# 23skdu/longbow

Hardware: AMD Instinct MI355X
Metric: k-NN queries/sec (batch=1024, k=100), 1Mx768 f32 (higher is better)
Workload: dtype f32

## Files before the change

### longbow_amd/build.py

```python
import os
import subprocess
import sys
from concurrent.futures import ThreadPoolExecutor

HERE = os.path.dirname(os.path.abspath(__file__))
CSRC = os.path.join(HERE, "csrc")
OUT = os.path.join(HERE, "liblongbow_gpu.so")
OUT_DIAG = os.path.join(HERE, "liblongbow_gpu_diag.so")
SOURCES = ["index.hip", "index_search.hip", "simd_api.hip", "pq.hip", "comm.hip", "flight.hip", "kernels_gemm.hip", "kernels_gemm_narrow.hip", "kernels_gemm_tall2.hip", "kernels_gemm_tall16.hip", "kernels_scan.hip", "kernels_select.hip", "kernels_finish.hip",
           "kernels_pq.hip", "kernels_pq2.hip", "kernels_filter.hip", "kernels_i8.hip"]
HEADERS = ["lb_device.h", "lb_exact.h", "lb_admit.h", "lb_host.h", "lb_index.h", "lb_combine.h", "lb_select.h", os.path.join("..", "..", "include", "longbow_gpu.h")]
HIPCC = os.environ.get("HIPCC", "/opt/rocm/bin/hipcc")
FLAGS = ["--offload-arch=gfx950", "-O3", "-std=c++17", "-fPIC", "-Wall", "-Wno-unused-function"]


def _stale(target, deps):
    if not os.path.exists(target):
        return True
    t = os.path.getmtime(target)
    return any(os.path.getmtime(d) > t for d in deps)


def build(force=False, verbose=False, diag=False):
    srcs = [s for s in SOURCES if os.path.exists(os.path.join(CSRC, s))]
    hdrs = [os.path.join(CSRC, h) for h in HEADERS]
    objs = []
    jobs = []
    out = OUT_DIAG if diag else OUT
    for s in srcs:
        src = os.path.join(CSRC, s)
        obj = os.path.join(CSRC, s.replace(".hip", ".diag.o" if diag else ".o"))
        objs.append(obj)
        if force or _stale(obj, [src] + hdrs):
            jobs.append([HIPCC] + FLAGS + (["-DLB_DIAG"] if diag else []) + ["-c", src, "-o", obj])

    def run(cmd):
        if verbose:
            print(" ".join(cmd), flush=True)
        r = subprocess.run(cmd, capture_output=True, text=True)
        if r.returncode != 0:
            raise RuntimeError("hipcc failed:\n" + " ".join(cmd) + "\n" + r.stdout + r.stderr)
        return r

    with ThreadPoolExecutor(max_workers=4) as ex:
        list(ex.map(run, jobs))
    if force or jobs or _stale(out, objs):
        run([HIPCC, "--offload-arch=gfx950", "-shared", "-fPIC", "-o", out] + objs + ["-ldl", "-lpthread"])
    return out


if __name__ == "__main__":
    print(build(force="--force" in sys.argv, verbose=True, diag="--diag" in sys.argv))
```

### longbow_amd/csrc/kernels_gemm.hip

```cpp
#include "lb_admit.h"

#include <cstdlib>

namespace lb {

constexpr int BM = 128;
constexpr int BN = 128;
constexpr int BK = 32;
constexpr int GEMM_THREADS = 256;

struct GemmArgs {
    const float *X;
    const float *norm2;
    const float *rnorm;
    int64_t row_begin, row_end;
    int D;
    const float *Q;
    int nq;
    const uint8_t *mask;
    const uint32_t *rowmap;
    CandState cs;
    int n_row_tiles, n_q_tiles;
    int boot;
};

__device__ __forceinline__ int swz_off(int row, int chunk)
{
    return row * BK + ((chunk ^ ((row >> 1) & 7)) << 2);
}

template <int MODE>
__device__ __forceinline__ f32x4 load_chunk(const float *base, int64_t row, int D, int k)
{
    f32x4 v = {0.f, 0.f, 0.f, 0.f};
    const float *p = base + row * (int64_t)D + k;
    if (MODE == 2) {
        v = *reinterpret_cast<const f32x4 *>(p);
    } else if (MODE == 1) {
        if (k < D) v = *reinterpret_cast<const f32x4 *>(p);
    } else {
        if (k + 0 < D) v.x = p[0];
        if (k + 1 < D) v.y = p[1];
        if (k + 2 < D) v.z = p[2];
        if (k + 3 < D) v.w = p[3];
    }
    return v;
}

template <int METRIC, int ALIGNED>
__global__ __launch_bounds__(GEMM_THREADS, 2) void gemm_filter_kernel(GemmArgs a)
{
    constexpr bool GLDS = ALIGNED == 2;
    const int b = blockIdx.x;
    const int xcd = b & 7;
    const int in_xcd = b >> 3;
    const int qt = in_xcd % a.n_q_tiles;
    const int rt = (in_xcd / a.n_q_tiles) * 8 + xcd;
    if (rt >= a.n_row_tiles) return;

    __shared__ __attribute__((aligned(16))) float lds_all[2 * 2 * BM * BK + BM + BM + BM / 4];
    float(*lds)[2][BM * BK] = reinterpret_cast<float(*)[2][BM * BK]>(lds_all);
    float *s_aux = lds_all + 2 * 2 * BM * BK;
    uint32_t *s_rowid = reinterpret_cast<uint32_t *>(s_aux + BM);
    uint8_t *s_vis = reinterpret_cast<uint8_t *>(s_rowid + BM);

    const int tid = threadIdx.x;
    const int lane = tid & 63;
    const int wave = tid >> 6;
    const int wr = wave >> 1, wc = wave & 1;
    const int l31 = lane & 31, h = lane >> 5;

    const int64_t row0 = a.row_begin + (int64_t)rt * BM;
    const int q0 = qt * BN;
    const int64_t last_row = a.row_end - 1;
    const int last_q = a.nq - 1;

    auto corpus_row = [&](int64_t pos) -> int64_t {
        if (pos > last_row) pos = last_row;
        return a.rowmap ? (int64_t)a.rowmap[pos] : pos;
    };
    const int64_t side_ri = corpus_row(row0 + (tid & (BM - 1)));

    int st_row[4], st_ch[4];
    int64_t st_xrow[4];
    int st_qrow[4];
#pragma unroll
    for (int i = 0; i < 4; i++) {
        int c = tid + GEMM_THREADS * i;
        st_row[i] = c >> 3;
        st_ch[i] = c & 7;
        st_xrow[i] = corpus_row(row0 + st_row[i]);
        int qr = q0 + st_row[i];
        st_qrow[i] = qr < last_q ? qr : last_q;
    }

    f32x16 acc[2][2];
#pragma unroll
    for (int i = 0; i < 2; i++)
#pragma unroll
        for (int j = 0; j < 2; j++)
#pragma unroll
            for (int r = 0; r < 16; r++) acc[i][j][r] = 0.f;

    const int nk = (a.D + BK - 1) / BK;
    f32x4 ra[4], rb[4];

    const float *gsrcA[4], *gsrcB[4];
    if (GLDS) {
#pragma unroll
        for (int i = 0; i < 4; i++) {
            const int j = wave * 4 + i;
            const int row = j * 8 + (lane >> 3);
            const int c = (lane & 7) ^ ((row >> 1) & 7);
            const int64_t xr = corpus_row(row0 + row);
            int qr = q0 + row;
            if (qr > last_q) qr = last_q;
            gsrcA[i] = a.X + xr * (int64_t)a.D + 4 * c;
            gsrcB[i] = a.Q + (int64_t)qr * a.D + 4 * c;
        }
    }
    const int wave_u = __builtin_amdgcn_readfirstlane(wave);
    auto glds_piece = [&](int p, int stage, int k0) {
        const int i = p >> 1;
        const int j = wave_u * 4 + i;
        if ((p & 1) == 0)
            __builtin_amdgcn_global_load_lds(
                (const __attribute__((address_space(1))) void *)(gsrcA[i] + k0),
                (__attribute__((address_space(3))) void *)(&lds[stage][0][j * 8 * BK]), 16, 0,
                2);
        else
            __builtin_amdgcn_global_load_lds(
                (const __attribute__((address_space(1))) void *)(gsrcB[i] + k0),
                (__attribute__((address_space(3))) void *)(&lds[stage][1][j * 8 * BK]), 16, 0, 0);
    };
    auto glds_stage = [&](int stage, int k0) {
#pragma unroll
        for (int p = 0; p < 8; p++) glds_piece(p, stage, k0);
    };
    if (GLDS) glds_stage(0, 0);
    const float aux_r = side_aux<METRIC>(a.norm2, a.rnorm, side_ri);
    uint8_t side_vis = 1;
    if (a.mask) side_vis = a.mask[side_ri];
    uint64_t tau_raw[2];
#pragma unroll
    for (int tn = 0; tn < 2; tn++) {
        const int qj = q0 + wc * 64 + tn * 32 + l31;
        tau_raw[tn] = lane_tau(a.cs.tau, qj, a.nq, a.boot);
    }
    if (tid < BM) {
        s_aux[tid] = aux_r;
        s_vis[tid] = (row0 + tid <= last_row && side_vis) ? (uint8_t)1 : (uint8_t)0;
        s_rowid[tid] = (uint32_t)side_ri;
    }
    float tau_key[2];
    uint32_t tau_row[2];
#pragma unroll
    for (int tn = 0; tn < 2; tn++) {
        tau_key[tn] = tau_key_of(tau_raw[tn]);
        tau_row[tn] = entry_row(tau_raw[tn]);
    }
    if (!GLDS) {
#pragma unroll
        for (int i = 0; i < 4; i++) {
            ra[i] = load_chunk<ALIGNED>(a.X, st_xrow[i], a.D, st_ch[i] * 4);
            rb[i] = load_chunk<ALIGNED>(a.Q, st_qrow[i], a.D, st_ch[i] * 4);
        }
#pragma unroll
        for (int i = 0; i < 4; i++) {
            *reinterpret_cast<f32x4 *>(&lds[0][0][swz_off(st_row[i], st_ch[i])]) = ra[i];
            *reinterpret_cast<f32x4 *>(&lds[0][1][swz_off(st_row[i], st_ch[i])]) = rb[i];
        }
    }
    __syncthreads();

    if constexpr (GLDS) {
        struct Frag {
            f32x4 a[2], b[2];
        };
        auto ldfrag = [&](Frag &f, int stage, int s) {
            const float *As = lds[stage][0];
            const float *Bs = lds[stage][1];
            const int ch = 2 * s + h;
#pragma unroll
            for (int t = 0; t < 2; t++) {
                f.a[t] = *reinterpret_cast<const f32x4 *>(&As[swz_off(wr * 64 + t * 32 + l31, ch)]);
                f.b[t] = *reinterpret_cast<const f32x4 *>(&Bs[swz_off(wc * 64 + t * 32 + l31, ch)]);
            }
        };
        auto mfma16 = [&](const Frag &f) {
#pragma unroll
            for (int e = 0; e < 4; e++)
#pragma unroll
                for (int tm = 0; tm < 2; tm++)
#pragma unroll
                    for (int tn = 0; tn < 2; tn++)
                        acc[tm][tn] = __builtin_amdgcn_mfma_f32_32x32x2f32(f.a[tm][e], f.b[tn][e], acc[tm][tn], 0, 0, 0);
        };
        Frag F0, F1;
        auto steps012 = [&](int cur) {
            ldfrag(F1, cur, 1);
            mfma16(F0);
            ldfrag(F0, cur, 2);
            mfma16(F1);
            ldfrag(F1, cur, 3);
            mfma16(F0);
#pragma unroll
            for (int s = 0; s < 3; s++) {
                __builtin_amdgcn_sched_group_barrier(0x008, 2, 0);
                __builtin_amdgcn_sched_group_barrier(0x100, 4, 0);
                __builtin_amdgcn_sched_group_barrier(0x008, 14, 0);
            }
            __builtin_amdgcn_sched_barrier(0);
        };
        ldfrag(F0, 0, 0);
        if (nk > 1) glds_stage(1, BK);
        int kt = 0;
        for (; kt + 2 < nk; kt++) {
            const int cur = kt & 1;
            steps012(cur);
            __syncthreads();
            const int k0 = (kt + 2) * BK;
            ldfrag(F0, cur ^ 1, 0);
#pragma unroll
            for (int p = 0; p < 8; p++) glds_piece(p, cur, k0);
            mfma16(F1);
            __builtin_amdgcn_sched_group_barrier(0x008, 2, 0);
            __builtin_amdgcn_sched_group_barrier(0x100, 4, 0);
#pragma unroll
            for (int p = 0; p < 7; p++) {
                __builtin_amdgcn_sched_group_barrier(0x020, 1, 0);
                __builtin_amdgcn_sched_group_barrier(0x008, 2, 0);
            }
            __builtin_amdgcn_sched_group_barrier(0x020, 1, 0);
        }
        if (kt + 1 < nk) {
            const int cur = kt & 1;
            steps012(cur);
            __syncthreads();
            ldfrag(F0, cur ^ 1, 0);
            mfma16(F1);
            __builtin_amdgcn_sched_group_barrier(0x008, 2, 0);
            __builtin_amdgcn_sched_group_barrier(0x100, 4, 0);
            __builtin_amdgcn_sched_group_barrier(0x008, 14, 0);
            kt++;
        }
        steps012(kt & 1);
        mfma16(F1);
    } else {
        for (int kt = 0; kt < nk; kt++) {
            const int cur = kt & 1;
            const bool has_next = kt + 1 < nk;
            if (has_next) {
                const int k0 = (kt + 1) * BK;
#pragma unroll
                for (int i = 0; i < 4; i++) {
                    ra[i] = load_chunk<ALIGNED>(a.X, st_xrow[i], a.D, k0 + st_ch[i] * 4);
                    rb[i] = load_chunk<ALIGNED>(a.Q, st_qrow[i], a.D, k0 + st_ch[i] * 4);
                }
            }
            const float *As = lds[cur][0];
            const float *Bs = lds[cur][1];
            f32x4 fa[2][2], fb[2][2];
#pragma unroll
            for (int t = 0; t < 2; t++) {
                fa[0][t] = *reinterpret_cast<const f32x4 *>(&As[swz_off(wr * 64 + t * 32 + l31, h)]);
                fb[0][t] = *reinterpret_cast<const f32x4 *>(&Bs[swz_off(wc * 64 + t * 32 + l31, h)]);
            }
#pragma unroll
            for (int s = 0; s < 4; s++) {
                const int cb = s & 1, nb = cb ^ 1;
                if (s < 3) {
                    const int ch = 2 * (s + 1) + h;
#pragma unroll
                    for (int t = 0; t < 2; t++) {
                        fa[nb][t] = *reinterpret_cast<const f32x4 *>(&As[swz_off(wr * 64 + t * 32 + l31, ch)]);
                        fb[nb][t] = *reinterpret_cast<const f32x4 *>(&Bs[swz_off(wc * 64 + t * 32 + l31, ch)]);
                    }
                }
#pragma unroll
                for (int e = 0; e < 4; e++)
#pragma unroll
                    for (int tm = 0; tm < 2; tm++)
#pragma unroll
                        for (int tn = 0; tn < 2; tn++)
                            acc[tm][tn] = __builtin_amdgcn_mfma_f32_32x32x2f32(fa[cb][tm][e], fb[cb][tn][e],
                                                                              acc[tm][tn], 0, 0, 0);
                if (s == 1 && has_next) {
                    const int nxt = cur ^ 1;
#pragma unroll
                    for (int i = 0; i < 4; i++) {
                        *reinterpret_cast<f32x4 *>(&lds[nxt][0][swz_off(st_row[i], st_ch[i])]) = ra[i];
                        *reinterpret_cast<f32x4 *>(&lds[nxt][1][swz_off(st_row[i], st_ch[i])]) = rb[i];
                    }
                }
            }
            __syncthreads();
        }
    }

    float aux[2][4][4];
    uint32_t rid[2][4][4];
    uint32_t vbits = 0;
#pragma unroll
    for (int tm = 0; tm < 2; tm++)
#pragma unroll
        for (int g = 0; g < 4; g++)
            vbits |= tile_rows4(s_aux, s_rowid, s_vis, wr * 64 + tm * 32 + 8 * g + 4 * h, aux[tm][g], rid[tm][g]) << (tm * 16 + g * 4);
#pragma unroll
    for (int tn = 0; tn < 2; tn++) {
        const int qj = q0 + wc * 64 + tn * 32 + l31;
        const bool qok = qj < a.nq;
        uint64_t *list = a.cs.lists + (size_t)(qok ? qj : 0) * a.cs.cap;
        if (a.boot) {
            if (qok) {
#pragma unroll
                for (int tm = 0; tm < 2; tm++)
#pragma unroll
                    for (int g = 0; g < 4; g++) {
                        const int64_t rbase = row0 + wr * 64 + tm * 32 + 8 * g + 4 * h;
                        uint64_t ent[4];
#pragma unroll
                        for (int e = 0; e < 4; e++)
                            ent[e] = ((vbits >> (tm * 16 + g * 4 + e)) & 1u) ? pack_entry(cand_key<METRIC>(acc[tm][tn][4 * g + e], aux[tm][g][e]), rid[tm][g][e]) : kEntryMax;
                        uint64_t *dst = list + (rbase - a.row_begin);
                        if (rbase + 3 < a.row_end) {
                            typedef unsigned long long u64x2 __attribute__((ext_vector_type(2)));
                            u64x2 v0 = {ent[0], ent[1]}, v1 = {ent[2], ent[3]};
                            *reinterpret_cast<u64x2 *>(dst) = v0;
                            *reinterpret_cast<u64x2 *>(dst + 2) = v1;
                        } else {
#pragma unroll
                            for (int e = 0; e < 4; e++)
                                if (rbase + e < a.row_end) dst[e] = ent[e];
                        }
                    }
            }
            continue;
        }
        uint32_t bits = 0;
#pragma unroll
        for (int tm = 0; tm < 2; tm++)
#pragma unroll
            for (int g = 0; g < 4; g++)
#pragma unroll
                for (int e = 0; e < 4; e++)
                    bits |= admit_exact(cand_key<METRIC>(acc[tm][tn][4 * g + e], aux[tm][g][e]), rid[tm][g][e], tau_key[tn], tau_row[tn]) << (tm * 16 + g * 4 + e);
        bits &= vbits;
        if (bits) {
            uint32_t pos = atomicAdd(&a.cs.cnt[qj], (uint32_t)__builtin_popcount(bits));
#pragma unroll
            for (int tm = 0; tm < 2; tm++)
#pragma unroll
                for (int g = 0; g < 4; g++)
#pragma unroll
                    for (int e = 0; e < 4; e++)
                        if (bits & (1u << (tm * 16 + g * 4 + e))) {
                            const uint32_t ri = rid[tm][g][e];
                            if (pos < a.cs.cap) list[pos] = pack_entry(cand_key<METRIC>(acc[tm][tn][4 * g + e], aux[tm][g][e]), ri);
                            pos++;
                        }
        }
    }
}

__global__ __launch_bounds__(256) void split_bf16_kernel(const float *src, float *dst, int64_t n8)
{
    for (int64_t i = (int64_t)blockIdx.x * blockDim.x + threadIdx.x; i < n8; i += (int64_t)gridDim.x * blockDim.x) {
        bf16x8 hi, lo;
        split_bf16x8(*reinterpret_cast<const f32x4 *>(src + i * 8), *reinterpret_cast<const f32x4 *>(src + i * 8 + 4), hi, lo);
        const int64_t grp = i >> 1;
        const int kb = (int)(i & 1);
        char *g = reinterpret_cast<char *>(dst) + grp * 64;
        *reinterpret_cast<bf16x8 *>(g + kb * 16) = hi;
        *reinterpret_cast<bf16x8 *>(g + 32 + kb * 16) = lo;
    }
}

void launch_split_bf16(const float *src, float *dst, int64_t rows, int D, hipStream_t s)
{
    const int64_t n8 = rows * (int64_t)D / 8;
    if (n8 <= 0) return;
    int64_t blocks = (n8 + 255) / 256;
    if (blocks > 16384) blocks = 16384;
    hipLaunchKernelGGL(split_bf16_kernel, dim3((unsigned)blocks), dim3(256), 0, s, src, dst, n8);
}

void launch_gemm_filter(int metric, const float *X, const float *norm2, const float *rnorm,
                        int64_t row_begin, int64_t row_end, int D, const float *Q, int nq,
                        const uint8_t *mask, const uint32_t *rowmap, CandState cs, bool boot, hipStream_t s)
{
    if (row_end <= row_begin || nq <= 0) return;
    GemmArgs a;
    a.rowmap = rowmap;
    a.boot = boot ? 1 : 0;
    a.X = X; a.norm2 = norm2; a.rnorm = rnorm;
    a.row_begin = row_begin; a.row_end = row_end; a.D = D;
    a.Q = Q; a.nq = nq; a.mask = mask; a.cs = cs;
    a.n_row_tiles = (int)((row_end - row_begin + BM - 1) / BM);
    a.n_q_tiles = (nq + BN - 1) / BN;
    const int groups = (a.n_row_tiles + 7) / 8;
    dim3 grid((unsigned)(groups * 8 * a.n_q_tiles));
    const bool aligned = (D % 4 == 0) && ((reinterpret_cast<uintptr_t>(X) & 15) == 0) &&
                         ((reinterpret_cast<uintptr_t>(Q) & 15) == 0);
    const int mode = !aligned ? 0 : (D % BK == 0 ? 2 : 1);
#define LB_GEMM(M, AL) hipLaunchKernelGGL((gemm_filter_kernel<M, AL>), grid, dim3(GEMM_THREADS), 0, s, a)
#define LB_GEMM_M(M)                 \
    do {                             \
        if (mode == 2) LB_GEMM(M, 2); \
        else if (mode == 1) LB_GEMM(M, 1); \
        else LB_GEMM(M, 0);           \
    } while (0)
    if (metric == METRIC_L2) LB_GEMM_M(METRIC_L2);
    else if (metric == METRIC_COS) LB_GEMM_M(METRIC_COS);
    else LB_GEMM_M(METRIC_DOT);
#undef LB_GEMM_M
#undef LB_GEMM
}

}
```

### longbow_amd/csrc/lb_device.h

```cpp
#pragma once
#include <hip/hip_runtime.h>
#include <stdint.h>
#include <stdlib.h>

namespace lb {

inline int lb_tunable(const char *name, int dflt)
{
#ifdef LB_DIAG
    const char *e = getenv(name);
    return e ? atoi(e) : dflt;
#else
    (void)name;
    return dflt;
#endif
}

constexpr uint64_t kEntryMax = ~0ull;

__host__ __device__ __forceinline__ uint32_t f32_sortable(float f)
{
    uint32_t u = __builtin_bit_cast(uint32_t, f);
    return (u & 0x80000000u) ? ~u : (u | 0x80000000u);
}
__host__ __device__ __forceinline__ float sortable_f32(uint32_t s)
{
    uint32_t u = (s & 0x80000000u) ? (s & 0x7fffffffu) : ~s;
    return __builtin_bit_cast(float, u);
}
__host__ __device__ __forceinline__ uint64_t pack_entry(float key, uint32_t row)
{
    key = key + 0.0f;
    const uint32_t sk = (key != key) ? 0xffc00000u  : f32_sortable(key);
    return ((uint64_t)sk << 32) | row;
}
__host__ __device__ __forceinline__ float entry_key(uint64_t e) { return sortable_f32((uint32_t)(e >> 32)); }
__host__ __device__ __forceinline__ uint32_t entry_row(uint64_t e) { return (uint32_t)e; }
__host__ __device__ __forceinline__ float tau_key_of(uint64_t tau)
{
    return tau == ~0ull ? __builtin_huge_valf() : entry_key(tau);
}

inline uint32_t next_pow2_host(uint32_t v)
{
    uint32_t p = 2;
    while (p < v) p <<= 1;
    return p;
}

inline int64_t chunk_end_host(int step, int64_t pos, int64_t n, int64_t keep, int64_t cap, bool safe,
                              bool big_boot = false)
{
    int64_t end;
    if (step == 0) {
        int64_t boot = 4 * keep > 2048 ? 4 * keep : 2048;
        if (boot > cap || big_boot) boot = cap;
        end = boot;
    } else if (safe) {
        end = pos + (cap - keep);
    } else {
        const int64_t target = (cap - keep) / 4;
        const double rows = (double)target * (double)pos / (double)(keep > 0 ? keep : 1);
        end = rows > 4e18 ? n : pos + (int64_t)rows;
        if (end <= pos) end = pos + 1;
        if (n - end < end - pos) end = n;
    }
    return end < n ? end : n;
}

enum : int { METRIC_L2 = 0, METRIC_COS = 1, METRIC_DOT = 2 };
enum : int { ORDER_SEQ = 0, ORDER_UNROLL4 = 1 };

struct CandState {
    uint64_t *lists;
    uint32_t *cnt;
    uint64_t *tau;
    uint32_t *flags;
    uint32_t cap;
    uint32_t *stripes;
};
constexpr int LB_STRIPES = 16;
constexpr int LB_STRIPE_PAD = 32;

#ifdef __HIPCC__
typedef float f32x4 __attribute__((ext_vector_type(4)));
typedef float f32x16 __attribute__((ext_vector_type(16)));
typedef __bf16 bf16x8 __attribute__((ext_vector_type(8)));
typedef _Float16 f16x8 __attribute__((ext_vector_type(8)));

template <bool NT>
__device__ __forceinline__ void lds_dma16x4(const void *g0, const void *g1, const void *g2, const void *g3, uint32_t lds_addr)
{
    uint32_t save;
    if (NT)
        asm volatile("s_mov_b32 %0, m0\n\ts_mov_b32 m0, %5\n\ts_nop 0\n\t"
                     "global_load_lds_dwordx4 %1, off nt\n\t"
                     "global_load_lds_dwordx4 %2, off offset:1024 nt\n\t"
                     "global_load_lds_dwordx4 %3, off offset:2048 nt\n\t"
                     "global_load_lds_dwordx4 %4, off offset:3072 nt\n\t"
                     "s_mov_b32 m0, %0"
                     : "=&s"(save) : "v"(g0), "v"(g1), "v"(g2), "v"(g3), "s"(lds_addr) : "memory");
    else
        asm volatile("s_mov_b32 %0, m0\n\ts_mov_b32 m0, %5\n\ts_nop 0\n\t"
                     "global_load_lds_dwordx4 %1, off\n\t"
                     "global_load_lds_dwordx4 %2, off offset:1024\n\t"
                     "global_load_lds_dwordx4 %3, off offset:2048\n\t"
                     "global_load_lds_dwordx4 %4, off offset:3072\n\t"
                     "s_mov_b32 m0, %0"
                     : "=&s"(save) : "v"(g0), "v"(g1), "v"(g2), "v"(g3), "s"(lds_addr) : "memory");
}
__device__ __forceinline__ void lds_dma16x2(const void *g0, const void *g1, uint32_t lds_addr)
{
    uint32_t save;
    asm volatile("s_mov_b32 %0, m0\n\ts_mov_b32 m0, %3\n\ts_nop 0\n\t"
                 "global_load_lds_dwordx4 %1, off\n\t"
                 "global_load_lds_dwordx4 %2, off offset:1024\n\t"
                 "s_mov_b32 m0, %0"
                 : "=&s"(save) : "v"(g0), "v"(g1), "s"(lds_addr) : "memory");
}
template <bool NT>
__device__ __forceinline__ void lds_dma16_noclobber(const void *g, uint32_t lds_addr)
{
    uint32_t save;
    if (NT)
        asm volatile("s_mov_b32 %0, m0\n\ts_mov_b32 m0, %2\n\ts_nop 0\n\t"
                     "global_load_lds_dwordx4 %1, off nt\n\t"
                     "s_mov_b32 m0, %0"
                     : "=&s"(save) : "v"(g), "s"(lds_addr));
    else
        asm volatile("s_mov_b32 %0, m0\n\ts_mov_b32 m0, %2\n\ts_nop 0\n\t"
                     "global_load_lds_dwordx4 %1, off\n\t"
                     "s_mov_b32 m0, %0"
                     : "=&s"(save) : "v"(g), "s"(lds_addr));
}
template <int N>
__device__ __forceinline__ void wait_vmcnt()
{
    __builtin_amdgcn_s_waitcnt((N & 15) | (7 << 4) | (15 << 8) | ((N >> 4) << 14));
    asm volatile("" ::: "memory");
}

__device__ __forceinline__ void split_bf16x8(const f32x4 x0, const f32x4 x1, bf16x8 &hi, bf16x8 &lo)
{
    const float x[8] = {x0.x, x0.y, x0.z, x0.w, x1.x, x1.y, x1.z, x1.w};
#pragma unroll
    for (int i = 0; i < 8; i++) {
        const __bf16 h = (__bf16)x[i];
        hi[i] = h;
        lo[i] = (__bf16)(x[i] - (float)h);
    }
}
__device__ __forceinline__ f16x8 cvt_f16x8(const f32x4 x0, const f32x4 x1)
{
    f16x8 r;
    r[0] = (_Float16)x0.x; r[1] = (_Float16)x0.y; r[2] = (_Float16)x0.z; r[3] = (_Float16)x0.w;
    r[4] = (_Float16)x1.x; r[5] = (_Float16)x1.y; r[6] = (_Float16)x1.z; r[7] = (_Float16)x1.w;
    return r;
}

template <int CTRL, int ROW_MASK>
__device__ __forceinline__ uint64_t dpp_u64(uint64_t v)
{
    const int lo = (int)(uint32_t)v, hi = (int)(uint32_t)(v >> 32);
    const int olo = __builtin_amdgcn_update_dpp(lo, lo, CTRL, ROW_MASK, 0xf, false);
    const int ohi = __builtin_amdgcn_update_dpp(hi, hi, CTRL, ROW_MASK, 0xf, false);
    return ((uint64_t)(uint32_t)ohi << 32) | (uint64_t)(uint32_t)olo;
}
template <int CTRL, int ROW_MASK>
__device__ __forceinline__ uint64_t min_dpp_u64(uint64_t v)
{
    const uint64_t o = dpp_u64<CTRL, ROW_MASK>(v);
    return o < v ? o : v;
}
__device__ __forceinline__ uint64_t row16_min_u64(uint64_t v)
{
    v = min_dpp_u64<0xB1, 0xf>(v);
    v = min_dpp_u64<0x4E, 0xf>(v);
    v = min_dpp_u64<0x141, 0xf>(v);
    v = min_dpp_u64<0x140, 0xf>(v);
    return v;
}
__device__ __forceinline__ uint64_t wave_min_u64(uint64_t v)
{
    v = row16_min_u64(v);
    v = min_dpp_u64<0x142, 0xa>(v);
    v = min_dpp_u64<0x143, 0xc>(v);
    const uint32_t lo = (uint32_t)__builtin_amdgcn_readlane((int)(uint32_t)v, 63);
    const uint32_t hi = (uint32_t)__builtin_amdgcn_readlane((int)(uint32_t)(v >> 32), 63);
    return ((uint64_t)hi << 32) | lo;
}

template <int CTRL, int ROW_MASK>
__device__ __forceinline__ uint32_t min_dpp_u32(uint32_t v)
{
    const uint32_t o = (uint32_t)__builtin_amdgcn_update_dpp((int)v, (int)v, CTRL, ROW_MASK, 0xf, false);
    return o < v ? o : v;
}
__device__ __forceinline__ uint32_t row16_min_u32(uint32_t v)
{
    v = min_dpp_u32<0xB1, 0xf>(v);
    v = min_dpp_u32<0x4E, 0xf>(v);
    v = min_dpp_u32<0x141, 0xf>(v);
    v = min_dpp_u32<0x140, 0xf>(v);
    return v;
}
__device__ __forceinline__ uint32_t wave_min_u32(uint32_t v)
{
    v = row16_min_u32(v);
    v = min_dpp_u32<0x142, 0xa>(v);
    v = min_dpp_u32<0x143, 0xc>(v);
    return (uint32_t)__builtin_amdgcn_readlane((int)v, 63);
}

#endif


void launch_row_norms(const float *X, int64_t n, int D, float *norm2, float *rnorm,
                      uint32_t *d_maxnorm2, hipStream_t s, const float *center = nullptr);
void launch_row_norms(const _Float16 *X, int64_t n, int D, float *norm2, float *rnorm, uint32_t *d_maxnorm2, hipStream_t s,
                      const float *center = nullptr);
void launch_widen_f16(const void *src, float *dst, int64_t n, hipStream_t s);

void launch_row_norms_i8(const int8_t *X, int64_t n, int D, int32_t *norm2, hipStream_t s);
void launch_widen_i8(const void *src, float *dst, int64_t n, hipStream_t s);
void launch_scan_i8(int metric, const int8_t *X, int64_t row_begin, int64_t row_end, int D, const float *Q, const int *qsel,
                    int nsel, const int32_t *norm2, const uint8_t *mask, const uint32_t *rowmap, CandState cs, bool boot,
                    hipStream_t s, bool striped);
void launch_sample_scores_i8(int metric, const int8_t *X, int D, int64_t span, uint32_t count, const uint32_t *rowmap,
                             const uint8_t *mask, const float *Q, const int *qsel, int nsel, CandState cs, hipStream_t s);
bool mfma_i8_supported(int metric, int D, const void *X, const void *Q8);
void launch_mfma_i8(int metric, const int8_t *X, int64_t npos, int D, const int8_t *Q8, int nq, const int32_t *qn,
                    const int32_t *norm2, const uint8_t *mask, const uint32_t *rowmap, CandState cs, bool sample, int64_t span,
                    hipStream_t s);
void launch_query_norms_i8(const int8_t *Q8, int nq, int D, int32_t *qn, hipStream_t s);
void launch_column_means(const float *X, int64_t n, int D, float *partial, float *center, int Dpad, hipStream_t s);
void launch_column_means(const _Float16 *X, int64_t n, int D, float *partial, float *center, int Dpad, hipStream_t s);

void launch_gemm_filter(int metric, const float *X, const float *norm2, const float *rnorm,
                        int64_t row_begin, int64_t row_end, int D, const float *Q, int nq,
                        const uint8_t *mask, const uint32_t *rowmap, CandState cs, bool boot, hipStream_t s);
void launch_gemm_filter_narrow(int metric, const float *X, const float *norm2, const float *rnorm,
                               int64_t row_begin, int64_t row_end, int D, const float *Q, int nq,
                               const uint8_t *mask, const uint32_t *rowmap, CandState cs, bool boot,
                               hipStream_t s, bool tile64 = false);
struct FusedSample {
    const uint32_t *smap = nullptr;
    uint32_t count = 0;
    int m = 0;
    uint32_t n_blocks = 0;
    uint32_t *ticket = nullptr;
    uint32_t ticket_base = 0;
    uint32_t *ready = nullptr;
    uint32_t epoch = 0;
    float *qna = nullptr;
    int order = 0;
    uint32_t *fail_host = nullptr;
};
void launch_gemm_filter_narrow_fused(int metric, const float *X, const float *norm2, const float *rnorm, int64_t row_begin,
                                     int64_t row_end, int D, const float *Q, int nq, const uint8_t *mask,
                                     const uint32_t *rowmap, CandState cs, hipStream_t s, bool tile64, FusedSample fs);
uint32_t fused_sample_blocks(uint32_t count, int nq, bool tile64);
void launch_split_bf16(const float *src, float *dst, int64_t rows, int D, hipStream_t s);
void launch_gemm_filter_tall2(int metric, const float *X, const float *norm2, const float *rnorm, int64_t row_begin,
                              int64_t row_end, int D, const float *Qs, int nq, const uint8_t *mask, const uint32_t *rowmap,
                              CandState cs, bool boot, int asplit, hipStream_t s);

struct Tall16Tin {
    uint32_t count;
    int m;
    uint32_t tag;
    uint32_t *fail_host;
    const float *Q;
    float *qna;
    int order;
#ifdef LB_DIAG
    int withhold;
#endif
};
bool tall16_tin_ok(int D, int nq, int64_t n_pos, bool img, bool mapped, bool masked, bool with_norm, uint32_t count, int m);
void launch_query_prep(const float *Q, int nq, int D, void *Qh, float *qinv, float *qna, int order, CandState cs, hipStream_t s,
                       const float *center = nullptr,
                       float *qnrm = nullptr,
                       bool tau_zero = false,
                       float *qrho = nullptr,
                       float rho_gain = 0.f);
void launch_gemm_filter_tall16(int metric, const float *X, const float *norm2, const float *rnorm, int64_t row_begin,
                               int64_t row_end, int D, const void *Qh, const float *qinv, int nq, const uint8_t *mask,
                               const uint32_t *rowmap, CandState cs, bool boot, hipStream_t s, const void *Xh = nullptr,
                               int64_t xh_cap = 0,
                               uint32_t gstride = 0,
                               const float *qnrm = nullptr, float gsum = 0.f,
                               const struct Tall16Tin *tin = nullptr);
void launch_corpus_to_f16(const float *X, int64_t row_begin, int64_t row_end, int D, void *Xh, int64_t cap, hipStream_t s,
                          const float *center = nullptr);
void launch_corpus_to_f16(const _Float16 *X, int64_t row_begin, int64_t row_end, int D, void *Xh, int64_t cap, hipStream_t s,
                          const float *center = nullptr);
void launch_f16_residual(const float *X, int64_t row_begin, int64_t row_end, int D, const float *center, uint32_t *stat, hipStream_t s);
void launch_f16_residual(const _Float16 *X, int64_t row_begin, int64_t row_end, int D, const float *center, uint32_t *stat, hipStream_t s);
int corpus_f16_plane_dims();
bool tall16_entries_are_positions(int D, int nq, bool img, bool mapped, bool masked);
bool tall16_runs_persistent(int D, int nq, bool img, bool mapped, bool masked);

struct EmitArgs {
    int k;
    const int64_t *ids;
    float *out_dist;
    int64_t *out_labels;
    uint32_t *flags_host;
};
void launch_select(CandState cs, const int *qsel, int nsel, int kc, uint32_t boot_rows, hipStream_t s,
                   uint32_t need_at_least = 0, const EmitArgs *emit = nullptr,
                   bool striped = false,
                   bool unsorted = false);
struct SamplePrep {
    void *Qh;
    float *qinv, *qnrm;
    const float *center;
    bool tau_zero;
    float *qrho;
    float rho_gain;
};
void launch_sample_scores(int metric, int order, const float *X, int D, int64_t span, uint32_t count,
                          const uint32_t *rowmap, const uint8_t *mask, const float *Q, const int *qsel, int nsel,
                          CandState cs, float *qna, hipStream_t s, const float *norm2 = nullptr,
                          const float *rnorm = nullptr,
                          const float *center = nullptr,
                          const SamplePrep *prep = nullptr);
void launch_sample_scores(int metric, int order, const _Float16 *X, int D, int64_t span, uint32_t count,
                          const uint32_t *rowmap, const uint8_t *mask, const float *Q, const int *qsel, int nsel,
                          CandState cs, float *qna, hipStream_t s, const float *norm2 = nullptr, const float *rnorm = nullptr,
                          const float *center = nullptr, const SamplePrep *prep = nullptr);
bool sample_tau_supported(uint32_t count, int m);
void launch_sample_tau(CandState cs, const int *qsel, int nsel, uint32_t count, int m, bool zero_stripes, hipStream_t s,
                       const float *Q = nullptr, int D = 0, float *qna = nullptr, int order = 0);
void launch_sample_map(const uint32_t *rowmap, int64_t span, uint32_t count, uint32_t *smap, hipStream_t s);

size_t finish_scratch_bytes(int nq_split_max, uint32_t smax);
void launch_finish(int metric, int order, const float *X, int D, const float *Q, int nq, const float *qna, CandState cs, int k,
                   const uint32_t *d_maxnorm2, float gamma, float beta, const int64_t *ids, const uint32_t *posmap, float *out_dist,
                   int64_t *out_labels, hipStream_t s, uint32_t *flags_host, uint32_t *done, uint32_t *xcnt, void *xscratch,
                   int nq_split_max, uint32_t smax,
                   const float *center = nullptr,
                   const float *lb_norm2 = nullptr, const float *lb_qnrm = nullptr, float lb_gsum = 0.f,
                   const float *qrho = nullptr, float qrho_k = 0.f);
void launch_finish(int metric, int order, const _Float16 *X, int D, const float *Q, int nq, const float *qna, CandState cs, int k,
                   const uint32_t *d_maxnorm2, float gamma, float beta, const int64_t *ids, const uint32_t *posmap, float *out_dist,
                   int64_t *out_labels, hipStream_t s, uint32_t *flags_host, uint32_t *done, uint32_t *xcnt, void *xscratch,
                   int nq_split_max, uint32_t smax,
                   const float *center = nullptr,
                   const float *lb_norm2 = nullptr, const float *lb_qnrm = nullptr, float lb_gsum = 0.f,
                   const float *qrho = nullptr, float qrho_k = 0.f);

void launch_query_norms(int order, const float *Q, const int *qsel, int nsel, int D, float *qna,
                        hipStream_t s);

void launch_scan(int metric, int order, bool raw_dot, const float *X, int64_t row_begin,
                 int64_t row_end, int D, const float *Q, const int *qsel, int nsel,
                 const float *qna, const uint8_t *mask, const uint32_t *rowmap, CandState cs, bool boot,
                 float *all_out, int64_t ld, hipStream_t s, bool striped = false);
void launch_scan(int metric, int order, bool raw_dot, const _Float16 *X, int64_t row_begin,
                 int64_t row_end, int D, const float *Q, const int *qsel, int nsel,
                 const float *qna, const uint8_t *mask, const uint32_t *rowmap, CandState cs, bool boot,
                 float *all_out, int64_t ld, hipStream_t s, bool striped = false);

void launch_emit_lists(CandState cs, const int *qsel, int nsel, int k, const int64_t *ids,
                       float *out_dist, int64_t *out_labels, uint32_t *flags_host, hipStream_t s);

void launch_init_cand(CandState cs, const int *qsel, int nsel, hipStream_t s);
void launch_fill_empty(float *dist, int64_t *lab, int64_t n, hipStream_t s);

void launch_merge_topk(int nshards, int64_t nq, int k, const float *dist_in, const int64_t *lab_in,
                       int64_t dist_stride, int64_t lab_stride, float *dist_out, int64_t *lab_out, hipStream_t s);

void launch_fill_uniform(float *dst, int64_t n, uint64_t seed, int64_t offset, hipStream_t s);
void launch_fill_codes(uint8_t *dst, int64_t n, uint64_t seed, int64_t offset, hipStream_t s);
void launch_fill_uniform_rows(float *dst, const int64_t *ids, int64_t nrows, int dim, uint64_t seed, hipStream_t s);

void launch_build_adc_table(const float *codebooks, int M, int K, int sub, const float *Q, int nq,
                            float *tables, hipStream_t s, float *minrng = nullptr,
                            uint32_t *zero_a = nullptr, uint32_t *zero_b = nullptr);
void launch_adc_scan(const float *table, int M, const uint8_t *codes, int64_t row_begin, int64_t row_end,
                     int slot, const uint8_t *mask, CandState cs, bool boot, float *all_out,
                     int64_t out_base, hipStream_t s, const int *skip_if_ok = nullptr);

void launch_adc_sample(const float *table, int M, const uint8_t *codes, int64_t n, uint32_t count, uint64_t *out,
                       hipStream_t s);
uint32_t launch_sample_topm(const uint64_t *in, uint32_t count_total, int m, CandState cs, int slot, hipStream_t s);

void launch_pq_encode(const float *codebooks, int M, int K, int sub, const float *X, int64_t n, uint8_t *codes,
                      hipStream_t s);
void launch_pq_decode(const float *codebooks, int M, int K, int sub, const uint8_t *codes, int64_t n, float *out,
                      hipStream_t s);
void launch_adc_quantise(const float *table, const float *minrng, int M, const uint64_t *tau, uint8_t *qtab, int *params,
                         hipStream_t s);
bool launch_adc_prefilter(const uint8_t *qtab, const int *params, int M, const uint8_t *codes, int64_t n,
                          uint32_t *cand, uint32_t cand_cap, uint32_t *cand_cnt, hipStream_t s);
bool launch_adc_prefilter2(const uint8_t *qtab, const int *params, uint32_t *cand, uint32_t *cand_cnt, const uint8_t *qtab2,
                           const int *params2, uint32_t *cand2, uint32_t *cand_cnt2, int M, const uint8_t *codes, int64_t n,
                           uint32_t cand_cap, hipStream_t s);
bool launch_adc_prefilter4(const uint8_t *const qtab[4], const int *const params[4], uint32_t *const cand[4], uint32_t *const cand_cnt[4],
                           int M, const uint8_t *codes, int64_t n, uint32_t cand_cap, hipStream_t s);
void launch_adc_exact_candidates(const float *table, int M, const uint8_t *codes, const uint32_t *cand,
                                 const uint32_t *cand_cnt, uint32_t cand_cap, const int *params, int slot, CandState cs,
                                 hipStream_t s);
void launch_adc_rerank(const float *table, int M, const uint8_t *codes, int64_t n, const int64_t *rows, int64_t nrows,
                       float *out_dist, float *out_score, hipStream_t s);

void launch_match_int64(const int64_t *src, int64_t n, int64_t val, int op, const uint8_t *validity,
                        int64_t valid_offset, uint8_t *dst, int combine, hipStream_t s);
void launch_match_float32(const float *src, int64_t n, float val, int op, const uint8_t *validity,
                          int64_t valid_offset, uint8_t *dst, int combine, hipStream_t s);
void launch_and_bytes(uint8_t *dst, const uint8_t *src, int64_t n, hipStream_t s);
int64_t compact_scratch_words(int64_t n);
void launch_compact_mask(const uint8_t *mask, int64_t n, uint32_t *rowmap, uint32_t *scratch, hipStream_t s);
void launch_rrf(int64_t nq, int kd, const int64_t *dense, int ks, const int64_t *sparse, int k, int limit,
                int64_t *out_ids, float *out_scores, hipStream_t s);

}
```

Measured before the change: 87280.

## Add persistent XCD-aware GEMM filter kernel with cross-tile prefetch pipeline

Adds a persistent version of the wide GEMM filter kernel. A fixed grid of 2 blocks per CU, grouped by XCD, loops over row/query tiles. The global-to-LDS double buffer runs across tile boundaries, and the side data for the next tile (norms, mask, rowids, tau) is prefetched during the current tile's k-loop. The aim is to hide the launch and tail cost, plus the per-tile pipeline fill and drain, and to improve L2 locality per XCD. It is used only for aligned D%32==0 non-boot calls with enough tiles, and it adds complexity around stale tau values and scheduling hints.

```diff
diff --git a/longbow_amd/build.py b/longbow_amd/build.py
--- a/longbow_amd/build.py
+++ b/longbow_amd/build.py
@@ -7,9 +7,9 @@
 CSRC = os.path.join(HERE, "csrc")
 OUT = os.path.join(HERE, "liblongbow_gpu.so")
 OUT_DIAG = os.path.join(HERE, "liblongbow_gpu_diag.so")
-SOURCES = ["index.hip", "index_search.hip", "simd_api.hip", "pq.hip", "comm.hip", "flight.hip", "kernels_gemm.hip", "kernels_gemm_narrow.hip", "kernels_gemm_tall2.hip", "kernels_gemm_tall16.hip", "kernels_scan.hip", "kernels_select.hip", "kernels_finish.hip",
+SOURCES = ["index.hip", "index_search.hip", "simd_api.hip", "pq.hip", "comm.hip", "flight.hip", "kernels_gemm.hip", "kernels_gemm_persist.hip", "kernels_gemm_narrow.hip", "kernels_gemm_tall2.hip", "kernels_gemm_tall16.hip", "kernels_scan.hip", "kernels_select.hip", "kernels_finish.hip",
            "kernels_pq.hip", "kernels_pq2.hip", "kernels_filter.hip", "kernels_i8.hip"]
-HEADERS = ["lb_device.h", "lb_exact.h", "lb_admit.h", "lb_host.h", "lb_index.h", "lb_combine.h", "lb_select.h", os.path.join("..", "..", "include", "longbow_gpu.h")]
+HEADERS = ["lb_device.h", "lb_exact.h", "lb_admit.h", "lb_gemm_wide.h", "lb_host.h", "lb_index.h", "lb_combine.h", "lb_select.h", os.path.join("..", "..", "include", "longbow_gpu.h")]
 HIPCC = os.environ.get("HIPCC", "/opt/rocm/bin/hipcc")
 FLAGS = ["--offload-arch=gfx950", "-O3", "-std=c++17", "-fPIC", "-Wall", "-Wno-unused-function"]
 
diff --git a/longbow_amd/csrc/kernels_gemm.hip b/longbow_amd/csrc/kernels_gemm.hip
--- a/longbow_amd/csrc/kernels_gemm.hip
+++ b/longbow_amd/csrc/kernels_gemm.hip
@@ -1,33 +1,8 @@
-#include "lb_admit.h"
+#include "lb_gemm_wide.h"
 
 #include <cstdlib>
 
 namespace lb {
-
-constexpr int BM = 128;
-constexpr int BN = 128;
-constexpr int BK = 32;
-constexpr int GEMM_THREADS = 256;
-
-struct GemmArgs {
-    const float *X;
-    const float *norm2;
-    const float *rnorm;
-    int64_t row_begin, row_end;
-    int D;
-    const float *Q;
-    int nq;
-    const uint8_t *mask;
-    const uint32_t *rowmap;
-    CandState cs;
-    int n_row_tiles, n_q_tiles;
-    int boot;
-};
-
-__device__ __forceinline__ int swz_off(int row, int chunk)
-{
-    return row * BK + ((chunk ^ ((row >> 1) & 7)) << 2);
-}
 
 template <int MODE>
 __device__ __forceinline__ f32x4 load_chunk(const float *base, int64_t row, int D, int k)
@@ -403,6 +378,13 @@
     const bool aligned = (D % 4 == 0) && ((reinterpret_cast<uintptr_t>(X) & 15) == 0) &&
                          ((reinterpret_cast<uintptr_t>(Q) & 15) == 0);
     const int mode = !aligned ? 0 : (D % BK == 0 ? 2 : 1);
+    if (mode == 2 && !boot) {
+        const int slots = gemm_persist_slots();
+        if (slots > 0 && (int64_t)a.n_row_tiles * a.n_q_tiles > 8 * (int64_t)slots) {
+            launch_gemm_filter_persist(metric, a, slots, s);
+            return;
+        }
+    }
 #define LB_GEMM(M, AL) hipLaunchKernelGGL((gemm_filter_kernel<M, AL>), grid, dim3(GEMM_THREADS), 0, s, a)
 #define LB_GEMM_M(M)                 \
     do {                             \
diff --git a/longbow_amd/csrc/kernels_gemm_persist.hip b/longbow_amd/csrc/kernels_gemm_persist.hip
--- /dev/null
+++ b/longbow_amd/csrc/kernels_gemm_persist.hip
@@ -0,0 +1,304 @@
+#include "lb_gemm_wide.h"
+
+namespace lb {
+
+constexpr int SIDE_WORDS = BM + BM + BM / 4;
+
+template <int METRIC>
+__global__ __launch_bounds__(GEMM_THREADS, 2) void gemm_filter_persist_kernel(GemmArgs a, int S)
+{
+    const int b = blockIdx.x;
+    const int xcd = b & 7;
+    const int slot = b >> 3;
+    const int lim = xcd < a.n_row_tiles ? ((a.n_row_tiles - xcd + 7) >> 3) * a.n_q_tiles : 0;
+    if (slot >= lim) return;
+    const int T = (lim - slot + S - 1) / S;
+
+    __shared__ __attribute__((aligned(16))) float lds_all[2 * 2 * BM * BK + 2 * SIDE_WORDS];
+    float(*lds)[2][BM * BK] = reinterpret_cast<float(*)[2][BM * BK]>(lds_all);
+    float *side = lds_all + 2 * 2 * BM * BK;
+
+    const int tid = threadIdx.x;
+    const int lane = tid & 63;
+    const int wave = tid >> 6;
+    const int wr = wave >> 1, wc = wave & 1;
+    const int l31 = lane & 31, h = lane >> 5;
+
+    const int64_t last_row = a.row_end - 1;
+    const int last_q = a.nq - 1;
+    const int nk = a.D / BK;
+    const int G = T * nk;
+
+    auto corpus_row = [&](int64_t pos) -> int64_t {
+        if (pos > last_row) pos = last_row;
+        return a.rowmap ? (int64_t)a.rowmap[pos] : pos;
+    };
+    auto tile_of = [&](int i, int &rt, int &qt) {
+        const int in_xcd = slot + i * S;
+        qt = in_xcd % a.n_q_tiles;
+        rt = (in_xcd / a.n_q_tiles) * 8 + xcd;
+    };
+
+    const float *gsrcA[4], *gsrcB[4];
+    int st_rt = -1, st_qt = -1;
+    auto set_pointers = [&](int i) {
+        int rt, qt;
+        tile_of(i, rt, qt);
+        if (rt != st_rt) {
+            const int64_t row0 = a.row_begin + (int64_t)rt * BM;
+#pragma unroll
+            for (int u = 0; u < 4; u++) {
+                const int row = (wave * 4 + u) * 8 + (lane >> 3);
+                const int c = (lane & 7) ^ ((row >> 1) & 7);
+                gsrcA[u] = a.X + corpus_row(row0 + row) * (int64_t)a.D + 4 * c;
+            }
+            st_rt = rt;
+        }
+        if (qt != st_qt) {
+            const int q0 = qt * BN;
+#pragma unroll
+            for (int u = 0; u < 4; u++) {
+                const int row = (wave * 4 + u) * 8 + (lane >> 3);
+                const int c = (lane & 7) ^ ((row >> 1) & 7);
+                int qr = q0 + row;
+                if (qr > last_q) qr = last_q;
+                gsrcB[u] = a.Q + (int64_t)qr * a.D + 4 * c;
+            }
+            st_qt = qt;
+        }
+    };
+    const int wave_u = __builtin_amdgcn_readfirstlane(wave);
+    auto glds_piece = [&](int p, int buf, int k0) {
+        const int u = p >> 1;
+        const int j = wave_u * 4 + u;
+        if ((p & 1) == 0)
+            __builtin_amdgcn_global_load_lds(
+                (const __attribute__((address_space(1))) void *)(gsrcA[u] + k0),
+                (__attribute__((address_space(3))) void *)(&lds[buf][0][j * 8 * BK]), 16, 0,
+                2);
+        else
+            __builtin_amdgcn_global_load_lds(
+                (const __attribute__((address_space(1))) void *)(gsrcB[u] + k0),
+                (__attribute__((address_space(3))) void *)(&lds[buf][1][j * 8 * BK]), 16, 0, 0);
+    };
+    int st_i = 0, st_k0 = 0;
+    auto advance = [&]() {
+        st_k0 += BK;
+        if (st_k0 >= a.D) {
+            st_k0 = 0;
+            st_i++;
+            if (st_i < T) set_pointers(st_i);
+        }
+    };
+
+    struct Side {
+        float aux;
+        uint32_t rowid;
+        uint8_t vis;
+        uint64_t tau[2];
+    };
+    auto fetch_side = [&](int i, Side &sd) {
+        int rt, qt;
+        tile_of(i, rt, qt);
+        const int64_t ri = corpus_row(a.row_begin + (int64_t)rt * BM + (tid & (BM - 1)));
+        sd.aux = side_aux<METRIC>(a.norm2, a.rnorm, ri);
+        sd.vis = 1;
+        if (a.mask) sd.vis = a.mask[ri];
+        sd.rowid = (uint32_t)ri;
+#pragma unroll
+        for (int tn = 0; tn < 2; tn++) {
+            const int qj = qt * BN + wc * 64 + tn * 32 + l31;
+            sd.tau[tn] = a.cs.tau[qj < last_q ? qj : last_q];
+        }
+    };
+    float tau_key[2];
+    uint32_t tau_row[2];
+    auto put_side = [&](int i, const Side &sd) {
+        int rt, qt;
+        tile_of(i, rt, qt);
+        float *s_aux = side + (i & 1) * SIDE_WORDS;
+        uint32_t *s_rowid = reinterpret_cast<uint32_t *>(s_aux + BM);
+        uint8_t *s_vis = reinterpret_cast<uint8_t *>(s_rowid + BM);
+        if (tid < BM) {
+            s_aux[tid] = sd.aux;
+            s_vis[tid] = (a.row_begin + (int64_t)rt * BM + tid <= last_row && sd.vis) ? (uint8_t)1 : (uint8_t)0;
+            s_rowid[tid] = sd.rowid;
+        }
+#pragma unroll
+        for (int tn = 0; tn < 2; tn++) {
+            const uint64_t tau = qt * BN + wc * 64 + tn * 32 + l31 < a.nq ? sd.tau[tn] : 0ull;
+            tau_key[tn] = tau_key_of(tau);
+            tau_row[tn] = entry_row(tau);
+        }
+    };
+
+    f32x16 acc[2][2];
+    auto zero_acc = [&]() {
+#pragma unroll
+        for (int i = 0; i < 2; i++)
+#pragma unroll
+            for (int j = 0; j < 2; j++)
+#pragma unroll
+                for (int r = 0; r < 16; r++) acc[i][j][r] = 0.f;
+    };
+    zero_acc();
+
+    struct Frag {
+        f32x4 a[2], b[2];
+    };
+    auto ldfrag = [&](Frag &f, int buf, int s) {
+        const float *As = lds[buf][0];
+        const float *Bs = lds[buf][1];
+        const int ch = 2 * s + h;
+#pragma unroll
+        for (int t = 0; t < 2; t++) {
+            f.a[t] = *reinterpret_cast<const f32x4 *>(&As[swz_off(wr * 64 + t * 32 + l31, ch)]);
+            f.b[t] = *reinterpret_cast<const f32x4 *>(&Bs[swz_off(wc * 64 + t * 32 + l31, ch)]);
+        }
+    };
+    auto mfma16 = [&](const Frag &f) {
+#pragma unroll
+        for (int e = 0; e < 4; e++)
+#pragma unroll
+            for (int tm = 0; tm < 2; tm++)
+#pragma unroll
+                for (int tn = 0; tn < 2; tn++)
+                    acc[tm][tn] = __builtin_amdgcn_mfma_f32_32x32x2f32(f.a[tm][e], f.b[tn][e], acc[tm][tn], 0, 0, 0);
+    };
+    Frag F0, F1;
+    auto steps012 = [&](int cur) {
+        ldfrag(F1, cur, 1);
+        mfma16(F0);
+        ldfrag(F0, cur, 2);
+        mfma16(F1);
+        ldfrag(F1, cur, 3);
+        mfma16(F0);
+#pragma unroll
+        for (int s = 0; s < 3; s++) {
+            __builtin_amdgcn_sched_group_barrier(0x008, 2, 0);
+            __builtin_amdgcn_sched_group_barrier(0x100, 4, 0);
+            __builtin_amdgcn_sched_group_barrier(0x008, 14, 0);
+        }
+        __builtin_amdgcn_sched_barrier(0);
+    };
+
+    auto epilogue = [&](int copy, int q0) {
+        const float *s_aux = side + copy * SIDE_WORDS;
+        const uint32_t *s_rowid = reinterpret_cast<const uint32_t *>(s_aux + BM);
+        const uint8_t *s_vis = reinterpret_cast<const uint8_t *>(s_rowid + BM);
+        float aux[2][4][4];
+        uint32_t rid[2][4][4];
+        uint32_t vbits = 0;
+#pragma unroll
+        for (int tm = 0; tm < 2; tm++)
+#pragma unroll
+            for (int g = 0; g < 4; g++)
+                vbits |= tile_rows4(s_aux, s_rowid, s_vis, wr * 64 + tm * 32 + 8 * g + 4 * h, aux[tm][g], rid[tm][g]) << (tm * 16 + g * 4);
+#pragma unroll
+        for (int tn = 0; tn < 2; tn++) {
+            const int qj = q0 + wc * 64 + tn * 32 + l31;
+            const bool qok = qj < a.nq;
+            uint64_t *list = a.cs.lists + (size_t)(qok ? qj : 0) * a.cs.cap;
+            uint32_t bits = 0;
+#pragma unroll
+            for (int tm = 0; tm < 2; tm++)
+#pragma unroll
+                for (int g = 0; g < 4; g++)
+#pragma unroll
+                    for (int e = 0; e < 4; e++)
+                        bits |= admit_exact(cand_key<METRIC>(acc[tm][tn][4 * g + e], aux[tm][g][e]), rid[tm][g][e], tau_key[tn], tau_row[tn]) << (tm * 16 + g * 4 + e);
+            bits &= vbits;
+            if (bits) {
+                uint32_t pos = atomicAdd(&a.cs.cnt[qj], (uint32_t)__builtin_popcount(bits));
+#pragma unroll
+                for (int tm = 0; tm < 2; tm++)
+#pragma unroll
+                    for (int g = 0; g < 4; g++)
+#pragma unroll
+                        for (int e = 0; e < 4; e++)
+                            if (bits & (1u << (tm * 16 + g * 4 + e))) {
+                                const uint32_t ri = rid[tm][g][e];
+                                if (pos < a.cs.cap) list[pos] = pack_entry(cand_key<METRIC>(acc[tm][tn][4 * g + e], aux[tm][g][e]), ri);
+                                pos++;
+                            }
+            }
+        }
+    };
+
+    set_pointers(0);
+#pragma unroll
+    for (int p = 0; p < 8; p++) glds_piece(p, 0, 0);
+    advance();
+    Side sd;
+    fetch_side(0, sd);
+    put_side(0, sd);
+    __syncthreads();
+    ldfrag(F0, 0, 0);
+    if (G > 1) {
+#pragma unroll
+        for (int p = 0; p < 8; p++) glds_piece(p, 1, st_k0);
+        advance();
+    }
+
+    const int fetch_kt = nk >= 2 ? nk - 2 : 0;
+    int i = 0, kt = 0;
+    for (int g = 0; g < G; g++) {
+        const int cur = g & 1;
+        steps012(cur);
+        __syncthreads();
+        if (g + 2 < G) {
+            ldfrag(F0, cur ^ 1, 0);
+#pragma unroll
+            for (int p = 0; p < 8; p++) glds_piece(p, cur, st_k0);
+            mfma16(F1);
+            __builtin_amdgcn_sched_group_barrier(0x008, 2, 0);
+            __builtin_amdgcn_sched_group_barrier(0x100, 4, 0);
+#pragma unroll
+            for (int p = 0; p < 7; p++) {
+                __builtin_amdgcn_sched_group_barrier(0x020, 1, 0);
+                __builtin_amdgcn_sched_group_barrier(0x008, 2, 0);
+            }
+            __builtin_amdgcn_sched_group_barrier(0x020, 1, 0);
+            advance();
+        } else {
+            ldfrag(F0, cur ^ 1, 0);
+            mfma16(F1);
+            __builtin_amdgcn_sched_group_barrier(0x008, 2, 0);
+            __builtin_amdgcn_sched_group_barrier(0x100, 4, 0);
+            __builtin_amdgcn_sched_group_barrier(0x008, 14, 0);
+        }
+        if (kt == fetch_kt && i + 1 < T) fetch_side(i + 1, sd);
+        if (++kt == nk) {
+            int rt, qt;
+            tile_of(i, rt, qt);
+            epilogue(i & 1, qt * BN);
+            if (i + 1 < T) put_side(i + 1, sd);
+            zero_acc();
+            kt = 0;
+            i++;
+        }
+    }
+}
+
+int gemm_persist_slots()
+{
+    static const int cus = [] {
+        int dev = 0, n = 0;
+        (void)hipGetDevice(&dev);
+        (void)hipDeviceGetAttribute(&n, hipDeviceAttributeMultiprocessorCount, dev);
+        return n;
+    }();
+    return 2 * cus / 8;
+}
+
+void launch_gemm_filter_persist(int metric, const GemmArgs &a, int slots, hipStream_t s)
+{
+    const dim3 grid((unsigned)(8 * slots));
+#define LB_GEMM_P(M) hipLaunchKernelGGL((gemm_filter_persist_kernel<M>), grid, dim3(GEMM_THREADS), 0, s, a, slots)
+    if (metric == METRIC_L2) LB_GEMM_P(METRIC_L2);
+    else if (metric == METRIC_COS) LB_GEMM_P(METRIC_COS);
+    else LB_GEMM_P(METRIC_DOT);
+#undef LB_GEMM_P
+}
+
+}
diff --git a/longbow_amd/csrc/lb_device.h b/longbow_amd/csrc/lb_device.h
--- a/longbow_amd/csrc/lb_device.h
+++ b/longbow_amd/csrc/lb_device.h
@@ -239,6 +239,9 @@
 void launch_gemm_filter(int metric, const float *X, const float *norm2, const float *rnorm,
                         int64_t row_begin, int64_t row_end, int D, const float *Q, int nq,
                         const uint8_t *mask, const uint32_t *rowmap, CandState cs, bool boot, hipStream_t s);
+struct GemmArgs;
+int gemm_persist_slots();
+void launch_gemm_filter_persist(int metric, const GemmArgs &a, int slots, hipStream_t s);
 void launch_gemm_filter_narrow(int metric, const float *X, const float *norm2, const float *rnorm,
                                int64_t row_begin, int64_t row_end, int D, const float *Q, int nq,
                                const uint8_t *mask, const uint32_t *rowmap, CandState cs, bool boot,
diff --git a/longbow_amd/csrc/lb_gemm_wide.h b/longbow_amd/csrc/lb_gemm_wide.h
--- /dev/null
+++ b/longbow_amd/csrc/lb_gemm_wide.h
@@ -0,0 +1,31 @@
+#pragma once
+#include "lb_admit.h"
+
+namespace lb {
+
+constexpr int BM = 128;
+constexpr int BN = 128;
+constexpr int BK = 32;
+constexpr int GEMM_THREADS = 256;
+
+struct GemmArgs {
+    const float *X;
+    const float *norm2;
+    const float *rnorm;
+    int64_t row_begin, row_end;
+    int D;
+    const float *Q;
+    int nq;
+    const uint8_t *mask;
+    const uint32_t *rowmap;
+    CandState cs;
+    int n_row_tiles, n_q_tiles;
+    int boot;
+};
+
+__device__ __forceinline__ int swz_off(int row, int chunk)
+{
+    return row * BK + ((chunk ^ ((row >> 1) & 7)) << 2);
+}
+
+}
```

Measured after the change: 77880. 10.8% lower.
